# jkflying/opencalibration

Hardware: AMD Instinct MI355X
Metric: images/sec end-to-end (extract+match+relax) on synthetic aerial grid; LM iters/sec (higher is better)
Workload: dtype f32 (extract) + fp4 0/1 bits, f32 accumulate, exact (match) + f64 (RANSAC, relax)

## Files before the change

### opencalibration_amd/csrc/akaze.hip

```cpp
#include "area_table.hpp"
#include "ctx.hpp"

#include <algorithm>
#include <cmath>
#include <limits>
#include <cstring>
#include <type_traits>
#include <vector>

namespace
{

struct level_info
{
    int octave, w, h, sigma_size;
    float esigma;
    size_t off;
    int tile_off, tiles_x;
    int mask_off;
    int sup_off, sup_tx;
};

__device__ __forceinline__ int clampi(int v, int lo, int hi)
{
// ... 2655 lines not shown
    if (!ctx || !images_dev || !cams || !model3 || !plane2 || !lattice3)
        return OCHIP_EINVAL;
    if (n_images == 0)
        return OCHIP_OK;
    OCHIP_HIP(ctx, hipSetDevice(ctx->device));
    std::vector<synth_cam> hc(n_images);
    for (uint32_t i = 0; i < n_images; i++)
    {
        for (int k = 0; k < 3; k++)
            hc[i].pos[k] = (float)cams[7 * i + k];
        for (int k = 0; k < 4; k++)
            hc[i].q[k] = (float)cams[7 * i + 3 + k];
    }
    synth_cam *dc = nullptr;
    if (hipMalloc((void **)&dc, n_images * sizeof(synth_cam)) != hipSuccess)
        return ochip_fail(ctx, OCHIP_ENOMEM, "hipMalloc failed");
    hipError_t e = hipMemcpy(dc, hc.data(), n_images * sizeof(synth_cam), hipMemcpyHostToDevice);
    if (e == hipSuccess)
    {
        hipLaunchKernelGGL(render_views_kernel, dim3((width + 255) / 256, height, n_images), dim3(256), 0, ctx->stream,
                           images_dev + (size_t)first_image * width * height * 3, width, height, (const synth_cam *)dc,
                           (float)model3[0], (float)model3[1], (float)model3[2], (float)plane2[0], (float)plane2[1],
                           (float)lattice3[0], (float)lattice3[1], (float)lattice3[2], seed);
        e = ochip_stream_wait(ctx, ctx->stream);
    }
    (void)hipFree(dc);
    if (e != hipSuccess)
        return ochip_fail(ctx, OCHIP_EHIP, "ochip_synth_render_views: %s", hipGetErrorString(e));
    return OCHIP_OK;
}

}

namespace
{

const gather_tab &host_gather_tab()
{
    static const gather_tab G = []() {
        gather_tab T{};
        static const float gauss25[7][7] = {{0.02546481f, 0.02350698f, 0.01849125f, 0.01239505f, 0.00708017f, 0.00344629f, 0.00142946f},
                                            {0.02350698f, 0.02169968f, 0.01706957f, 0.01144208f, 0.00653582f, 0.00318132f, 0.00131956f},
                                            {0.01849125f, 0.01706957f, 0.01342740f, 0.00900066f, 0.00514126f, 0.00250252f, 0.00103800f},
                                            {0.01239505f, 0.01144208f, 0.00900066f, 0.00603332f, 0.00344629f, 0.00167749f, 0.00069579f},
                                            {0.00708017f, 0.00653582f, 0.00514126f, 0.00344629f, 0.00196855f, 0.00095820f, 0.00039744f},
                                            {0.00344629f, 0.00318132f, 0.00250252f, 0.00167749f, 0.00095820f, 0.00046640f, 0.00019346f},
                                            {0.00142946f, 0.00131956f, 0.00103800f, 0.00069579f, 0.00039744f, 0.00019346f, 0.00008024f}};
        std::vector<float> gw(169);
        for (int i = -6; i <= 6; i++)
            for (int j = -6; j <= 6; j++)
                gw[(i + 6) * 13 + (j + 6)] = gauss25[std::abs(i)][std::abs(j)];
        struct os
        {
            int q, i, j;
        };
        std::vector<os> S;
        int q = 0;
        for (int i = -6; i <= 6; i++)
            for (int j = -6; j <= 6; j++)
                if (i * i + j * j < 36)
                    S.push_back({q++, i, j});
        std::sort(S.begin(), S.end(), [](const os &a, const os &b) { return a.j != b.j ? a.j < b.j : a.i < b.i; });
        for (int L = 0; L < 128; L++)
        {
            T.ori[L] = 0xFFFFFFFFu;
            T.ori_g[L] = 0.0f;
// ... 38 lines not shown
                if (i < 6)
                    k = i;
                for (int ch = 0; ch < 3; ch++)
                    T.bit_ofs[3 * i + ch] = (unsigned int)((cell_of(full[k][0], full[k][1]) * 3 + channel_of[ch]) * 4) |
                                            ((unsigned int)((cell_of(full[k][0], full[k][2]) * 3 + channel_of[ch]) * 4) << 16);
                for (int q = 0; q < 3; q++)
                    full[k][q] = full[162 - i - 1][q];
            }
        }
        for (int i = 0; i < 64; i++)
            T.chain[i] = 3u << 11;
        struct ch_t
        {
            int cls, first_cell, i, j, follows;
        };
        std::vector<ch_t> chains;
        for (int k = 0; k < 4; k++)
            chains.push_back({0, k, -10 + (k / 2) * 10, -10 + (k % 2) * 10, 0});
        for (int k = 0; k < 9; k += 2)
            chains.push_back({1, 4 + k, -10 + (k / 3) * 7, -10 + (k % 3) * 7, k == 2 ? 1 : 0});
        for (int k = 0; k < 16; k += 4)
            chains.push_back({2, 13 + k, -10 + (k / 4) * 5, -10, 0});
        for (size_t cidx = 0; cidx < chains.size(); cidx++)
            for (int ch = 0; ch < 3; ch++)
            {
                const ch_t &cc = chains[cidx];
                const unsigned int p0 = (unsigned int)((cc.i + 10) * 21 + (cc.j + 10));
                T.chain[3 * cidx + ch] = p0 | ((unsigned int)ch << 9) | ((unsigned int)cc.cls << 11) |
                                         ((unsigned int)cc.first_cell << 13) | ((unsigned int)cc.follows << 18);
            }
        return T;
    }();
    return G;
}

int akaze_run(ochip_ctx *ctx, const uint8_t *images_bgr, bool on_device, uint32_t n_images, int width, int height,
              uint32_t max_kp, float *kp6, uint64_t *desc, uint32_t *counts, int *work_wh, const ochip_feature_lists *lists,
              double nms_radius)
{
    if (!ctx || !counts || (n_images && (!images_bgr || (!lists && (!kp6 || !desc)))))
        return OCHIP_EINVAL;
    if (width <= 0 || height <= 0)
        return ochip_fail(ctx, OCHIP_EINVAL, "bad image size %d x %d", width, height);
    OCHIP_HIP(ctx, hipSetDevice(ctx->device));
    hipStream_t st = ctx->stream;
    const double scale = std::min(1.f, float(1600) / (float)std::max(width, height));
    const int W = (int)std::lrint(width * scale), H = (int)std::lrint(height * scale);
    if (work_wh)
    {
        work_wh[0] = W;
        work_wh[1] = H;
    }
    for (uint32_t i = 0; i < n_images; i++)
        counts[i] = 0;
    if (n_images == 0)
        return OCHIP_OK;

    const int omax = 4, nsub = 4;
    const float soffset = 1.6f, dfactor = 1.5f, dthreshold = 0.00005f;
    levels_dev LV{};
    std::vector<std::vector<float>> tsteps;
    size_t img_stride = 0;
    int n_tiles = 0;
    size_t mask_stride = 0;
    size_t sup_stride = 0;
    {
// ... 23 lines not shown
                l.sup_tx = (lw + 7) / 8;
                sup_stride += (size_t)l.sup_tx * ((lh + 7) / 8);
                etime.push_back(0.5f * (l.esigma * l.esigma));
            }
        }
        tsteps.resize(LV.n);
        for (int i = 1; i < LV.n; i++)
            tsteps[i] = fed_taus(etime[i] - etime[i - 1], 0.25f);
    }
    const size_t plane0 = (size_t)W * H;
    const uint32_t B = n_images;
    const uint32_t max_cands = std::max<uint32_t>(max_kp * 4, 1u << 16);

    ochip::dev_scratch mem{ctx, "akaze"};
    constexpr auto WAIT = ochip::copy_mode::enqueue_wait;
    int rc = OCHIP_OK;
#define AK(call)                                                                                                       \
    do                                                                                                                 \
    {                                                                                                                  \
        if (rc == OCHIP_OK)                                                                                            \
            rc = (call);                                                                                               \
    } while (0)
    uint8_t *d_bgr = nullptr, *d_gray = nullptr;
    float *d_img = nullptr, *d_flow = nullptr, *d_ping = nullptr;
    float2 *d_Lxy = nullptr;
    float2 *d_Fit = nullptr;
    float *d_Lt = nullptr, *d_Rmax = nullptr, *d_kc = nullptr,
          *d_kp = nullptr;
    unsigned int *d_hmax = nullptr, *d_hist = nullptr, *d_ncand = nullptr, *d_pmax = nullptr;
    cand_t *d_cands = nullptr;
    unsigned char *d_dead = nullptr, *d_valid = nullptr;
    unsigned long long *d_desc = nullptr, *d_descc = nullptr;
    float *d_kpc = nullptr;
    unsigned int *d_counts = nullptr, *d_tile_counts = nullptr, *d_tile_base = nullptr, *d_tile_seq = nullptr;
    unsigned long long *d_mask = nullptr, *d_vmask = nullptr, *d_kmask = nullptr, *d_pmask = nullptr, *d_rmask = nullptr;
    unsigned int *d_found = nullptr;
    unsigned int *d_level_first = nullptr;
    unsigned int *d_turns = nullptr, *d_waiting = nullptr;
    unsigned int *d_wbase = nullptr, *d_live = nullptr, *d_nlive = nullptr;
    gather_tab *d_gtab = nullptr;
    const size_t src_px = (size_t)width * height;
    auto tiles = [&](int w, int h) { return dim3(8 * ((((w + BT_X - 1) / BT_X) * ((h + BT_Y - 1) / BT_Y) + 7) / 8), 1, B); };
    auto det_tiles = [&](int w, int h) { return dim3(8 * ((((w + BT_X - 1) / BT_X) * ((h + DT_Y - 1) / DT_Y) + 7) / 8), 1, B); };
    const dim3 tiles0 = tiles(W, H);
    const int n_tiles0 = ((W + BT_X - 1) / BT_X) * ((H + BT_Y - 1) / BT_Y);
    if (on_device)
        d_bgr = const_cast<uint8_t *>(images_bgr);
    else
        AK(mem.upload(&d_bgr, images_bgr, (size_t)B * src_px * 3, WAIT));
    AK(mem.alloc<uint8_t>(&d_gray, (size_t)B * src_px + 4));
    AK(mem.alloc<float>(&d_img, (size_t)B * plane0));
    AK(mem.alloc<float>(&d_flow, (size_t)B * plane0));
    AK(mem.alloc<float>(&d_ping, (size_t)B * plane0));
    AK(mem.alloc<unsigned int>(&d_pmax, (size_t)B * n_tiles0));
    AK(mem.alloc<float>(&d_Lt, (size_t)B * img_stride));
    AK(mem.alloc<float2>(&d_Lxy, (size_t)B * img_stride));
    AK(mem.alloc<float2>(&d_Fit, (size_t)B * img_stride));
    AK(mem.alloc<float>(&d_Rmax, (size_t)B * img_stride));
    AK(mem.alloc<float>(&d_kc, B));
    AK(mem.alloc<unsigned int>(&d_hmax, B));
    AK(mem.alloc<unsigned int>(&d_hist, (size_t)B * 301));
    AK(mem.alloc<unsigned int>(&d_ncand, B));
    AK(mem.alloc<cand_t>(&d_cands, (size_t)B * max_cands));
    AK(mem.alloc<unsigned char>(&d_dead, (size_t)B * max_cands));
    AK(mem.alloc<unsigned char>(&d_valid, (size_t)B * max_cands));
    AK(mem.alloc<float>(&d_kp, (size_t)B * max_cands * 6));
    AK(mem.alloc<unsigned long long>(&d_desc, (size_t)B * max_cands * 8));
    AK(mem.alloc<float>(&d_kpc, (size_t)B * max_kp * 6));
    AK(mem.alloc<unsigned long long>(&d_descc, (size_t)B * max_kp * 8));
    AK(mem.alloc<unsigned int>(&d_counts, B));
    AK(mem.alloc<unsigned int>(&d_tile_counts, (size_t)B * n_tiles));
    AK(mem.alloc<unsigned int>(&d_tile_base, (size_t)B * n_tiles));
    AK(mem.alloc<unsigned long long>(&d_mask, (size_t)B * mask_stride));
    AK(mem.alloc<unsigned long long>(&d_vmask, (size_t)B * mask_stride));
    AK(mem.alloc<unsigned long long>(&d_kmask, (size_t)B * sup_stride));
    AK(mem.alloc<unsigned long long>(&d_pmask, (size_t)B * sup_stride));
    AK(mem.alloc<unsigned long long>(&d_rmask, (size_t)B * sup_stride));
    AK(mem.alloc<unsigned int>(&d_turns, (size_t)B * 2 * max_cands));
    AK(mem.alloc<unsigned int>(&d_waiting, (size_t)B * LV.n));
    AK(mem.alloc<unsigned int>(&d_level_first, (size_t)B * (LV.n + 1)));
    AK(mem.alloc<unsigned int>(&d_found, (size_t)B * max_cands));
    AK(mem.alloc<unsigned int>(&d_wbase, (size_t)B * mask_stride));
    AK(mem.alloc<unsigned int>(&d_live, (size_t)B * max_cands));
    AK(mem.alloc<unsigned int>(&d_nlive, B));
    {
        std::vector<std::pair<uint64_t, unsigned int>> keyed;
        keyed.reserve(n_tiles);
        auto spread = [](uint32_t v) {
            uint64_t x = v;
            x = (x | (x << 16)) & 0x0000FFFF0000FFFFull;
            x = (x | (x << 8)) & 0x00FF00FF00FF00FFull;
            x = (x | (x << 4)) & 0x0F0F0F0F0F0F0F0Full;
            x = (x | (x << 2)) & 0x3333333333333333ull;
            x = (x | (x << 1)) & 0x5555555555555555ull;
            return x;
        };
        for (int i = 0; i < LV.n; i++)
        {
            const level_info &l = LV.l[i];
            const int ty_n = (l.h + DT_Y - 1) / DT_Y;
            for (int ty = 0; ty < ty_n; ty++)
                for (int tx = 0; tx < l.tiles_x; tx++)
                    keyed.emplace_back(((uint64_t)i << 48) | spread((uint32_t)tx) | (spread((uint32_t)ty) << 1),
                                       (unsigned int)(l.tile_off + ty * l.tiles_x + tx));
        }
        std::sort(keyed.begin(), keyed.end());
        std::vector<unsigned int> seq(keyed.size());
        for (size_t i = 0; i < keyed.size(); i++)
            seq[i] = keyed[i].second;
        AK(mem.upload(&d_tile_seq, seq.data(), seq.size(), WAIT));
    }
    {
        AK(mem.upload(&d_gtab, &host_gather_tab(), 1, WAIT));
    }
    if (rc != OCHIP_OK)
    return rc;
    auto grid2 = [&](int w, int h) { return dim3((w + 255) / 256, h, B); };
    auto taps_of = [](const std::vector<float> &k) {
        taps_t t{};
        t.n = (int)k.size();
        for (int i = 0; i < t.n && i < MAX_TAPS; i++)
            t.k[i] = k[i];
        return t;
    };
    const taps_t g1 = taps_of(gaussian_taps(1.0f)), g0 = taps_of(gaussian_taps(soffset));
    if (g1.n != 5 || g0.n != 9)
    return ochip_fail(ctx, OCHIP_EINVAL, "akaze: unexpected Gaussian kernel sizes %d / %d", g1.n, g0.n);
    hipEvent_t e0, e1;
    ochip_prof_begin(ctx, OCHIP_K_AKAZE, &e0, &e1);

    const size_t n_px = (size_t)B * src_px;
    const bool resized = !(W == width && H == height);
    area_tab tx, ty;
    bool staged = false;
    if (resized)
    {
        tx = area_table(width, W, 1.0 / scale);
        ty = area_table(height, H, 1.0 / scale);
        staged = width % 4 == 0;
        for (int x0 = 0; x0 < W && staged; x0 += 256)
        {
            const int x1 = std::min(x0 + 256, W);
            const int c0 = tx.si[tx.off[x0]] & ~3, c1 = tx.si[tx.off[x1] - 1];
            staged = c1 - c0 + 1 <= RS_PITCH - 3;
            for (int x = x0; x < x1 && staged; x++)
                staged = tx.off[x + 1] - tx.off[x] <= RESIZE_MAX_TAPS;
        }
        for (int y0 = 0; y0 < H && staged; y0 += RESIZE_ROWS)
        {
            const int y1 = std::min(y0 + RESIZE_ROWS, H);
            staged = ty.si[ty.off[y1] - 1] - ty.si[ty.off[y0]] + 1 <= RS_ROWS;
        }
    }
    const bool fused_grey = staged && ((uintptr_t)d_bgr & 3) == 0;
    if (!fused_grey)
    {
        if (((uintptr_t)d_bgr & 3) == 0)
            hipLaunchKernelGGL(gray4_kernel, dim3((unsigned)(((n_px + 3) / 4 + 255) / 256)), dim3(256), 0, st,
                               (const uint32_t *)d_bgr, (uint32_t *)d_gray, n_px / 4);
        if (((uintptr_t)d_bgr & 3) != 0 || (n_px & 3))
        {
            const size_t first = ((uintptr_t)d_bgr & 3) ? 0 : (n_px & ~(size_t)3);
            hipLaunchKernelGGL(gray_kernel, dim3((unsigned)((n_px - first + 255) / 256)), dim3(256), 0, st, d_bgr + 3 * first,
                               d_gray + first, n_px - first);
        }
    }
    if (W == width && H == height)
        hipLaunchKernelGGL(to_float_kernel, dim3((unsigned)((B * plane0 + 255) / 256)), dim3(256), 0, st, d_gray, d_img,
                           B * plane0);
    else
    {
        int *xo, *xs, *yo, *ys;
        float *xa, *ya;
        AK(mem.upload(&xo, tx.off.data(), tx.off.size(), WAIT));
        AK(mem.upload(&xs, tx.si.data(), tx.si.size(), WAIT));
        AK(mem.upload(&xa, tx.alpha.data(), tx.alpha.size(), WAIT));
        AK(mem.upload(&yo, ty.off.data(), ty.off.size(), WAIT));
        AK(mem.upload(&ys, ty.si.data(), ty.si.size(), WAIT));
        AK(mem.upload(&ya, ty.alpha.data(), ty.alpha.size(), WAIT));
        if (rc != OCHIP_OK)
        return rc;
        const dim3 rgrid((W + 255) / 256, (H + RESIZE_ROWS - 1) / RESIZE_ROWS, B);
        int most_taps = 0;
        for (int x = 0; x < W; x++)
            most_taps = std::max(most_taps, tx.off[x + 1] - tx.off[x]);
        const int half_up_cols = scale == 0.5 ? W - W % 16 : 0;
        if (fused_grey && most_taps <= 4)
            hipLaunchKernelGGL((resize_area_lds_kernel<true, 4>), rgrid, dim3(256), 0, st, (const uint8_t *)d_bgr, width, height, d_img,
                               W, H, xo, xs, xa, yo, ys, ya, half_up_cols);
        else if (fused_grey)
            hipLaunchKernelGGL((resize_area_lds_kernel<true, RESIZE_MAX_TAPS>), rgrid, dim3(256), 0, st, (const uint8_t *)d_bgr, width, height, d_img,
                               W, H, xo, xs, xa, yo, ys, ya, half_up_cols);
        else if (staged)
            hipLaunchKernelGGL((resize_area_lds_kernel<false, RESIZE_MAX_TAPS>), rgrid, dim3(256), 0, st, d_gray, width, height, d_img, W, H, xo, xs,
                               xa, yo, ys, ya, half_up_cols);
        else
            hipLaunchKernelGGL(resize_area_kernel, rgrid, dim3(256), 0, st, d_gray, width, height, d_img, W, H, xo, xs, xa, yo, ys,
                               ya, half_up_cols);
    }

    OCHIP_HIP(ctx, hipMemsetAsync(d_hist, 0, (size_t)B * 301 * 4, st));
    const bool modg_tiles = ochip_test_hook("tile_levels"), modg_force = ochip_test_hook("strip_levels");
    const bool modg_strip = !modg_tiles && (W & 1) == 0 && (plane0 & 1) == 0 && W >= 64 && H >= 64 && ((uintptr_t)d_img & 15) == 0 &&
                            ((uintptr_t)d_flow & 15) == 0 && (modg_force || (size_t)W * H * B >= ((size_t)32 << 20));
    if (modg_strip)
    {
        OCHIP_HIP(ctx, hipMemsetAsync(d_hmax, 0, (size_t)B * 4, st));
        level_strip_args sa{};
        sa.in = d_img, sa.in_stride = plane0;
        sa.flow = d_flow, sa.flow_stride = plane0;
        sa.w = W, sa.h = H;
        sa.hmax_bits = d_hmax;
        for (int q = 0; q < 5; q++)
            sa.k[q] = g1.k[q];
        typedef level_strip_geom<2, 0> MG;
        const int strips = ((W + MG::OW - 1) / MG::OW) * ((H + MG::H - 1) / MG::H);
        hipLaunchKernelGGL((level_strip_kernel<2, 0, true, true>), dim3(8 * (((strips + 3) / 4 + 7) / 8), 1, B), dim3(256), 0, st, sa);
    }
// ... 426 lines not shown
```

### opencalibration_amd/csrc/ctx.hip

```cpp
#include "ctx.hpp"

#include <cstring>

static std::string g_create_error;

int ochip_fail(ochip_ctx *ctx, int code, const char *fmt, ...)
{
    char buf[512];
    va_list ap;
    va_start(ap, fmt);
    vsnprintf(buf, sizeof buf, fmt, ap);
    va_end(ap);
    if (ctx)
        ctx->error = buf;
    else
        g_create_error = buf;
    return code;
}

int ochip_ensure(ochip_ctx *ctx, void **ptr, size_t *cap, size_t bytes)
{
    if (bytes <= *cap)
        return OCHIP_OK;
    if (*ptr)
// ... 78 lines not shown
        ochip_fail(ctx, OCHIP_ENOMEM, "device allocation of %zu bytes failed in %s", bytes, what);
    return d;
}

int dev_blocks::upload_bytes(void **dst, const void *src, size_t bytes, copy_mode m)
{
    void *d = get(bytes);
    if (!d)
        return OCHIP_ENOMEM;
    if (src && bytes)
    {
        hipError_t e = m == copy_mode::blocking ? hipMemcpy(d, src, bytes, hipMemcpyHostToDevice)
                                                : hipMemcpyAsync(d, src, bytes, hipMemcpyHostToDevice, ctx->stream);
        if (e == hipSuccess && m == copy_mode::enqueue_wait)
            e = ochip_stream_wait(ctx, ctx->stream);
        if (e != hipSuccess)
            return ochip_fail(ctx, OCHIP_EHIP, "host-to-device copy of %zu bytes failed in %s: %s", bytes, what, hipGetErrorString(e));
    }
    *dst = d;
    return OCHIP_OK;
}

void dev_blocks::release()
{
    for (auto &b : held)
        ochip_pool_put(ctx, b.first, b.second);
    held.clear();
}

dev_scratch::~dev_scratch()
{
    if (held.empty())
        return;
    (void)ochip_stream_wait(ctx, ctx->stream);
    release();
}
}

void ochip_prof_begin(ochip_ctx *ctx, int kid, hipEvent_t *start, hipEvent_t *stop)
{
    auto &s = ctx->prof[kid];
    if (!s.free_list.empty())
    {
        *start = s.free_list.back().first;
        *stop = s.free_list.back().second;
        s.free_list.pop_back();
    }
    else
    {
        (void)hipEventCreate(start);
        (void)hipEventCreate(stop);
    }
    (void)hipEventRecord(*start, ctx->stream);
}

static void prof_drain(ochip_ctx *ctx, int kid)
{
    auto &s = ctx->prof[kid];
    for (auto &p : s.pending)
    {
        float ms = 0;
        (void)hipEventSynchronize(p.second);
        if (hipEventElapsedTime(&ms, p.first, p.second) == hipSuccess)
        {
            s.total_ms += ms;
            s.launches++;
        }
        s.free_list.push_back(p);
    }
    s.pending.clear();
}

void ochip_prof_end(ochip_ctx *ctx, int kid, hipEvent_t start, hipEvent_t stop)
{
    (void)hipEventRecord(stop, ctx->stream);
    auto &s = ctx->prof[kid];
    s.pending.emplace_back(start, stop);
    if (s.pending.size() >= 4096)
        prof_drain(ctx, kid);
}

extern "C"
{

int ochip_ctx_create(int device, ochip_ctx **out)
{
    if (!out)
        return ochip_fail(nullptr, OCHIP_EINVAL, "out is NULL");
    *out = nullptr;
    int count = 0;
    if (hipGetDeviceCount(&count) != hipSuccess || count <= 0)
        return ochip_fail(nullptr, OCHIP_ENODEV, "no HIP device visible");
    if (device < 0 || device >= count)
        return ochip_fail(nullptr, OCHIP_EINVAL, "device %d out of range (0..%d)", device, count - 1);
    ochip_ctx *ctx = new (std::nothrow) ochip_ctx();
    if (!ctx)
        return ochip_fail(nullptr, OCHIP_ENOMEM, "host allocation failed");
    ctx->device = device;
    hipError_t e = hipSetDevice(device);
    const char *bsync = getenv("OCHIP_BLOCKING_SYNC");
    ctx->blocking_wait = !(bsync && bsync[0] == '0');
    if (e == hipSuccess && ctx->blocking_wait)
    {
        (void)hipSetDeviceFlags(hipDeviceScheduleBlockingSync);
        (void)hipGetLastError();
    }
    if (e == hipSuccess)
        e = hipGetDeviceProperties(&ctx->prop, device);
    if (e == hipSuccess && std::strncmp(ctx->prop.gcnArchName, "gfx950", 6) != 0)
    {
        int rc = ochip_fail(nullptr, OCHIP_ENODEV, "device %d is %s; libochip is built for gfx950 only", device,
                            ctx->prop.gcnArchName);
        delete ctx;
        return rc;
    }
    if (e == hipSuccess)
        e = hipStreamCreateWithFlags(&ctx->stream, hipStreamNonBlocking);
    if (e != hipSuccess)
    {
        int rc = ochip_fail(nullptr, OCHIP_EHIP, "context creation failed: %s", hipGetErrorString(e));
        delete ctx;
        return rc;
    }
    *out = ctx;
    return OCHIP_OK;
}

void ochip_ctx_destroy(ochip_ctx *ctx)
{
    if (!ctx)
        return;
    if (ctx->attachment && ctx->attachment_destroy)
        ctx->attachment_destroy(ctx->attachment);
    ctx->attachment = nullptr;
    for (ochip_ctx *sib : ctx->siblings)
        ochip_ctx_destroy(sib);
    ctx->siblings.clear();
    (void)hipSetDevice(ctx->device);
    (void)hipDeviceSynchronize();
    for (auto &s : ctx->prof)
    {
        for (auto &p : s.pending)
            s.free_list.push_back(p);
        for (auto &p : s.free_list)
        {
            (void)hipEventDestroy(p.first);
            (void)hipEventDestroy(p.second);
        }
    }
    void *bufs[] = {ctx->desc_dev,      ctx->img_off_dev,   ctx->img_n_dev, ctx->pairs_dev,    ctx->out_off_dev,
                    ctx->match_out_dev, ctx->kp_xy_dev,     ctx->rays_dev,  ctx->kp_image_dev, ctx->models_dev,
                    ctx->ms_recs_dev,   ctx->ms_seg_dev,    ctx->ms_flag_dev};
    for (void *b : bufs)
        if (b)
            (void)hipFree(b);
    for (void *b : ctx->scratch_dev)
        if (b)
            (void)hipFree(b);
    if (ctx->sym_jobs_dev)
        (void)hipFree(ctx->sym_jobs_dev);
    if (ctx->sym_part_dev)
        (void)hipFree(ctx->sym_part_dev);
    for (void *b : {ctx->desc_fp4_dev, ctx->desc_negpop_dev, ctx->desc_pop_dev})
        if (b)
            (void)hipFree(b);
    if (ctx->lab_table_mem)
    {
        ctx->lab_table_mem->release();
        delete ctx->lab_table_mem;
    }
    for (auto &b : ctx->dev_pool)
        (void)hipFree(b.first);
    for (auto &b : ctx->pinned_pool)
        (void)hipHostFree(b.first);
    for (auto &b : ctx->pinned_live)
        (void)hipHostFree(b.first);
    if (ctx->sync_event)
        (void)hipEventDestroy(ctx->sync_event);
    for (hipStream_t r : ctx->retired_streams)
        (void)hipStreamDestroy(r);
    if (ctx->stream)
        (void)hipStreamDestroy(ctx->stream);
    if (ctx->copy_stream)
        (void)hipStreamDestroy(ctx->copy_stream);
    delete ctx;
}

int ochip_ctx_set_priority(ochip_ctx *ctx, int high)
{
    if (!ctx)
        return OCHIP_EINVAL;
    if (ctx->stream_priority == (high ? 1 : 0))
        return OCHIP_OK;
    OCHIP_HIP(ctx, hipSetDevice(ctx->device));
    int least = 0, greatest = 0;
    OCHIP_HIP(ctx, hipDeviceGetStreamPriorityRange(&least, &greatest));
    OCHIP_HIP(ctx, hipStreamSynchronize(ctx->stream));
    hipStream_t s = nullptr;
    OCHIP_HIP(ctx, hipStreamCreateWithPriority(&s, hipStreamNonBlocking, high ? greatest : least));
    ctx->retired_streams.push_back(ctx->stream);
    ctx->stream = s;
    ctx->stream_priority = high ? 1 : 0;
    return OCHIP_OK;
}

int ochip_ctx_sibling(ochip_ctx *ctx, uint32_t index, ochip_ctx **out)
{
    if (!ctx || !out)
        return OCHIP_EINVAL;
    *out = nullptr;
    std::lock_guard<std::mutex> lock(ctx->siblings_mutex);
    if (index > 64)
        return ochip_fail(ctx, OCHIP_EINVAL, "sibling index %u out of range", index);
    while (ctx->siblings.size() <= index)
    {
        ochip_ctx *s = nullptr;
        const int rc = ochip_ctx_create(ctx->device, &s);
        if (rc != OCHIP_OK)
            return ochip_fail(ctx, rc, "sibling context: %s", ochip_last_error(nullptr));
        ctx->siblings.push_back(s);
    }
    *out = ctx->siblings[index];
    return OCHIP_OK;
}

void *ochip_ctx_attachment(ochip_ctx *ctx, void *(*make)(void), void (*destroy)(void *))
{
    if (!ctx)
        return nullptr;
    std::lock_guard<std::mutex> lock(ctx->siblings_mutex);
    if (!ctx->attachment && make)
    {
        ctx->attachment = make();
        ctx->attachment_destroy = destroy;
    }
    return ctx->attachment;
}

uint64_t ochip_akaze_progress(const ochip_ctx *ctx)
{
    return ctx ? ctx->akaze_readbacks.load(std::memory_order_acquire) : 0;
}

const char *ochip_last_error(const ochip_ctx *ctx)
{
    return ctx ? ctx->error.c_str() : g_create_error.c_str();
}

int ochip_device_info(const ochip_ctx *ctx, char *name, size_t name_len, int *compute_units, size_t *hbm_bytes)
{
    if (!ctx)
        return OCHIP_EINVAL;
    if (name && name_len)
        snprintf(name, name_len, "%s (%s)", ctx->prop.name[0] ? ctx->prop.name : "AMD Instinct (name table not installed)",
                 ctx->prop.gcnArchName);
    if (compute_units)
        *compute_units = ctx->prop.multiProcessorCount;
    if (hbm_bytes)
        *hbm_bytes = ctx->prop.totalGlobalMem;
    return OCHIP_OK;
}

int ochip_synchronize(ochip_ctx *ctx)
{
    if (!ctx)
        return OCHIP_EINVAL;
    OCHIP_HIP(ctx, ochip_stream_wait(ctx, ctx->stream));
    if (ctx->copy_stream)
        OCHIP_HIP(ctx, ochip_stream_wait(ctx, ctx->copy_stream));
    return OCHIP_OK;
}

int ochip_descriptors_reserve(ochip_ctx *ctx, uint32_t n_images, uint64_t total_descriptors)
{
    if (!ctx)
        return OCHIP_EINVAL;
    OCHIP_HIP(ctx, hipSetDevice(ctx->device));
    OCHIP_HIP(ctx, ochip_stream_wait(ctx, ctx->stream));
    ctx->kp_set.clear();
    ctx->rays_dirty = false;
    ctx->kp_store_ready = false;
    ctx->desc_capacity = ctx->desc_used = 0;
    ctx->fp4_valid = 0;
    ctx->n_images = n_images;
    ctx->img_off.assign(n_images, 0);
    ctx->img_n.assign(n_images, 0);
    ctx->img_set.assign(n_images, 0);
    ctx->img_tables_dirty = true;
    const size_t n_img = n_images ? n_images : 1;
    int rc = ochip_ensure(ctx, (void **)&ctx->desc_dev, &ctx->desc_bytes, (size_t)(total_descriptors ? total_descriptors : 1) * 64);
    if (rc == OCHIP_OK)
        rc = ochip_ensure(ctx, (void **)&ctx->img_off_dev, &ctx->img_off_bytes, n_img * 8);
    if (rc == OCHIP_OK)
        rc = ochip_ensure(ctx, (void **)&ctx->img_n_dev, &ctx->img_n_bytes, n_img * 4);
    if (rc != OCHIP_OK)
        return rc;
    ctx->desc_capacity = total_descriptors;
    return OCHIP_OK;
}

// ... 97 lines not shown
{
    if (!ctx || !p)
        return;
    for (size_t i = 0; i < ctx->pinned_live.size(); i++)
        if (ctx->pinned_live[i].first == p)
        {
            ctx->pinned_pool.push_back(ctx->pinned_live[i]);
            ctx->pinned_live.erase(ctx->pinned_live.begin() + i);
            while (ctx->pinned_pool.size() > 16)
            {
                size_t s = 0;
                for (size_t k = 1; k < ctx->pinned_pool.size(); k++)
                    if (ctx->pinned_pool[k].second < ctx->pinned_pool[s].second)
                        s = k;
                (void)hipHostFree(ctx->pinned_pool[s].first);
                ctx->pinned_pool.erase(ctx->pinned_pool.begin() + s);
            }
            return;
        }
}

int ochip_descriptor_count(const ochip_ctx *ctx, uint32_t image_id, uint32_t *n)
{
    if (!ctx || !n || image_id >= ctx->n_images || !ctx->img_set[image_id])
        return OCHIP_EINVAL;
    *n = ctx->img_n[image_id];
    return OCHIP_OK;
}

int ochip_profile_reset(ochip_ctx *ctx)
{
    if (!ctx)
        return OCHIP_EINVAL;
    OCHIP_HIP(ctx, ochip_stream_wait(ctx, ctx->stream));
    for (int k = 0; k < OCHIP_K_COUNT; k++)
    {
        prof_drain(ctx, k);
        ctx->prof[k].launches = 0;
        ctx->prof[k].total_ms = 0;
    }
    ctx->match_computed = ctx->match_delivered = 0;
    ctx->relax_mfma_flops = 0;
    ctx->ransac_hyp_corr = ctx->relax_blocks_jac = ctx->relax_blocks_cost = 0;
    for (ochip_ctx *sib : ctx->siblings)
    {
        const int rc = ochip_profile_reset(sib);
        if (rc != OCHIP_OK)
            return rc;
    }
    return OCHIP_OK;
}

int ochip_relax_work(ochip_ctx *ctx, double *mfma_flops)
{
    if (!ctx || !mfma_flops)
        return OCHIP_EINVAL;
    *mfma_flops = ctx->relax_mfma_flops;
    for (ochip_ctx *sib : ctx->siblings)
        *mfma_flops += sib->relax_mfma_flops;
    return OCHIP_OK;
}

int ochip_work_counters(ochip_ctx *ctx, uint64_t *counters3)
{
    if (!ctx || !counters3)
        return OCHIP_EINVAL;
    counters3[0] = ctx->ransac_hyp_corr;
// ... 73 lines not shown
```

### opencalibration_amd/csrc/ctx.hpp

```cpp
#pragma once

#include <hip/hip_runtime.h>

#include <atomic>
#include <cstdarg>
#include <cstdio>
#include <mutex>
#include <string>
#include <vector>

#include "../../include/ochip.h"
#include "env.hpp"

struct ochip_profile_slot
{
    std::vector<std::pair<hipEvent_t, hipEvent_t>> pending;
    std::vector<std::pair<hipEvent_t, hipEvent_t>> free_list;
    uint64_t launches = 0;
    double total_ms = 0;
};

namespace ochip
{
struct dev_blocks;
}

struct ochip_ctx
{
    int device = 0;
    hipStream_t stream = nullptr;
    hipStream_t copy_stream = nullptr;
    std::vector<hipStream_t> retired_streams;
    int stream_priority = -1;
    hipEvent_t sync_event = nullptr;
    bool blocking_wait = true;
    std::string error;
    hipDeviceProp_t prop{};

    uint32_t *desc_dev = nullptr;
    uint64_t desc_capacity = 0, desc_used = 0;
    uint32_t n_images = 0;
    std::vector<uint64_t> img_off;
    std::vector<uint32_t> img_n;
    std::vector<uint8_t> img_set;
    uint64_t *img_off_dev = nullptr;
    uint32_t *img_n_dev = nullptr;
    bool img_tables_dirty = true;

    double *kp_xy_dev = nullptr;
    double *rays_dev = nullptr;
    uint32_t *kp_image_dev = nullptr;
    double *models_dev = nullptr;
    std::vector<uint8_t> kp_set;
    bool rays_dirty = false;
    bool kp_store_ready = false;
    size_t desc_bytes = 0, img_off_bytes = 0, img_n_bytes = 0, kp_xy_bytes = 0, rays_bytes = 0, kp_image_bytes = 0,
           models_bytes = 0;

    ochip_pair *pairs_dev = nullptr;
    uint64_t *out_off_dev = nullptr;
    size_t pairs_cap = 0;
    ochip_match *match_out_dev = nullptr;
    size_t match_out_cap = 0;
    uint64_t match_out_total = 0;
    void *ms_recs_dev = nullptr, *ms_seg_dev = nullptr, *ms_flag_dev = nullptr;
    size_t ms_recs_cap = 0, ms_seg_cap = 0, ms_flag_cap = 0;
    uint32_t ms_pairs = 0;
    void *sym_jobs_dev = nullptr, *sym_part_dev = nullptr;
    size_t sym_jobs_cap = 0, sym_part_cap = 0;
    void *desc_fp4_dev = nullptr, *desc_negpop_dev = nullptr, *desc_pop_dev = nullptr;
    size_t desc_fp4_cap = 0, desc_negpop_cap = 0, desc_pop_cap = 0;
    uint64_t fp4_valid = 0;

    void *scratch_dev[8] = {nullptr};
    size_t scratch_cap[8] = {0};

    std::vector<std::pair<void *, size_t>> pinned_live, pinned_pool;
    std::vector<std::pair<void *, size_t>> dev_pool;

    ochip_profile_slot prof[OCHIP_K_COUNT];
    uint64_t match_computed = 0, match_delivered = 0;
    double relax_mfma_flops = 0;
    uint64_t ransac_hyp_corr = 0, relax_blocks_jac = 0, relax_blocks_cost = 0;
    uint64_t relax_system_bytes = 0, relax_system_dense_bytes = 0, relax_system_unknowns = 0;

    std::vector<ochip_ctx *> siblings;
    std::mutex siblings_mutex;

    std::atomic<uint64_t> akaze_readbacks{0};

    ochip::dev_blocks *lab_table_mem = nullptr;
    uint32_t *lab_table_dev = nullptr;
    void *lab_tables_dev = nullptr;
    float lab_table_fill_ms = 0;

    void *attachment = nullptr;
    void (*attachment_destroy)(void *) = nullptr;
};


inline hipError_t ochip_stream_wait(ochip_ctx *ctx, hipStream_t st)
{
    if (!ctx->blocking_wait)
        return hipStreamSynchronize(st);
    if (!ctx->sync_event)
    {
        const hipError_t e = hipEventCreateWithFlags(&ctx->sync_event, hipEventBlockingSync | hipEventDisableTiming);
        if (e != hipSuccess)
            return e;
    }
    const hipError_t e = hipEventRecord(ctx->sync_event, st);
    return e != hipSuccess ? e : hipEventSynchronize(ctx->sync_event);
}

inline hipError_t ochip_copy_stream(ochip_ctx *ctx, hipStream_t *out)
{
    hipError_t e = hipSuccess;
    if (!ctx->copy_stream)
        e = hipStreamCreateWithFlags(&ctx->copy_stream, hipStreamNonBlocking);
    *out = ctx->copy_stream;
    return e;
}

int ochip_fail(ochip_ctx *ctx, int code, const char *fmt, ...);
int ochip_ensure(ochip_ctx *ctx, void **ptr, size_t *cap, size_t bytes);
int ochip_ensure_keypoint_store(ochip_ctx *ctx, size_t n_keypoints, size_t n_images);
void *ochip_pool_get(ochip_ctx *ctx, size_t bytes, size_t *got);
void ochip_pool_put(ochip_ctx *ctx, void *p, size_t bytes);
void ochip_prof_begin(ochip_ctx *ctx, int kid, hipEvent_t *start, hipEvent_t *stop);
void ochip_prof_end(ochip_ctx *ctx, int kid, hipEvent_t start, hipEvent_t stop);

#define OCHIP_HIP(ctx, call)                                                                                           \
    do                                                                                                                 \
    {                                                                                                                  \
        hipError_t e__ = (call);                                                                                       \
// ... 72 lines not shown
```

### opencalibration_amd/csrc/host/extract_features.cpp

```cpp
#include "../env.hpp"
#include "extract_features.hpp"
#include "extract_slots.hpp"
#include "sort_like_std.hpp"

#include <algorithm>
#include <chrono>
#include <cmath>
#include <condition_variable>
#include <cstdio>
#include <cstdlib>
#include <cstring>
#include <deque>
#include <limits>
#include <mutex>
#include <thread>

#include <emmintrin.h>
#include <omp.h>

namespace opencalibration_amd
{

namespace
{
// ... 268 lines not shown
            g_tail_prof[i] += d[i];
        }
    }
}

struct chunk_buffers
{
    float *kp = nullptr;
    uint64_t *desc = nullptr;
    uint8_t *prepared = nullptr;
    ochip_feature_lists lists{};
    std::vector<uint32_t> counts;
    uint32_t first = 0, n = 0;
};

extract_slots &slots_of(ochip_ctx *root)
{
    void *p = ochip_ctx_attachment(
        root, []() -> void * { return new extract_slots(); }, [](void *q) { delete static_cast<extract_slots *>(q); });
    return *static_cast<extract_slots *>(p);
}

extract_slots::order handover_order()
{
    const char *gate = std::getenv("OCHIP_EXTRACT_GATE");
    if (gate && gate[0] == '0')
        return extract_slots::order::none;
    const char *e = std::getenv("OCHIP_EXTRACT_HANDOVER");
    if (e && std::strcmp(e, "survey") == 0)
        return extract_slots::order::survey;
    return extract_slots::order::slot;
}

bool stagger_starts()
{
    const char *e = std::getenv("OCHIP_EXTRACT_STAGGER");
    return e && e[0] == '1';
}
}

uint32_t extract_chunk_size()
{
    if (const char *e = std::getenv("OCHIP_EXTRACT_CHUNK"))
    {
        const long v = std::atol(e);
        if (v >= 1 && v <= 1024)
            return (uint32_t)v;
    }
    return 100;
}

std::vector<extracted_features> extract_features_batch(ochip_ctx *ctx, const uint8_t *images_bgr, uint32_t n_images,
                                                       int width, int height, uint32_t max_keypoints, std::string *error,
                                                       bool images_on_device)
{
    std::vector<extracted_features> out(n_images);
    const bool ok = extract_features_stream(ctx, images_bgr, n_images, width, height, max_keypoints, images_on_device, 0,
                                            [&](uint32_t first, uint32_t count, extracted_features *f) {
                                                for (uint32_t i = 0; i < count; i++)
                                                    out[first + i] = std::move(f[i]);
                                            },
                                            error);
    if (!ok)
        return {};
    return out;
}

bool extract_features_stream(ochip_ctx *ctx, const uint8_t *images_bgr, uint32_t n_images, int width, int height,
                             uint32_t max_keypoints, bool images_on_device, int host_threads,
                             const std::function<void(uint32_t, uint32_t, extracted_features *)> &on_chunk,
                             std::string *error, extract_timing *timing)
{
    if (timing)
        *timing = extract_timing{};
    if (n_images == 0)
        return true;
    if (width <= 0 || height <= 0)
    {
        std::vector<extracted_features> empty(n_images);
        on_chunk(0, n_images, empty.data());
        return true;
    }
    const int tail_threads = host_threads > 0 ? host_threads : omp_get_max_threads();
    const int max_length_pixels = 1600;
    const double scale = std::min(1.f, float(max_length_pixels) / (float)std::max(width, height));
    const uint32_t host_chunk = 25;
    const uint32_t chunk = std::min(images_on_device ? extract_chunk_size() : host_chunk, n_images);
    const size_t image_bytes = (size_t)width * height * 3;

    uint32_t n_drivers = images_on_device ? 4 : 5;
    if (const char *e = std::getenv("OCHIP_EXTRACT_STREAMS"))
        n_drivers = (uint32_t)std::max(1L, std::min(5L, std::atol(e)));
    const uint32_t n_chunks = (n_images + chunk - 1) / chunk;
    n_drivers = std::min(n_drivers, n_chunks);
    std::vector<ochip_ctx *> ctxs(n_drivers, ctx);
    for (uint32_t d = 1; d < n_drivers; d++)
        if (ochip_ctx_sibling(ctx, d - 1, &ctxs[d]) != OCHIP_OK)
        {
            if (error)
                *error = std::string("ochip_ctx_sibling: ") + ochip_last_error(ctx);
            return false;
        }
    const bool device_tail = !ochip_test_hook("host_tail");
    const double nms_pixel_radius = 8;
    const bool force_host_nms = ochip_test_hook("host_nms");
    extract_slots &slots = slots_of(ctx);
    const extract_slots::order handover = handover_order();
    const auto t_enter = std::chrono::steady_clock::now();
    extract_ticket ticket(slots, n_drivers);
    constexpr int BPS = extract_slots::BUFFERS_PER_SLOT;
    const uint32_t n_bufs = BPS * n_drivers;
    std::vector<chunk_buffers> bufs(n_bufs);
    std::string fail;
    const size_t rows = (size_t)chunk * max_keypoints;
    const size_t o_resp = (rows + chunk) * 88, o_slot = o_resp + rows * 4, o_ns = o_slot + rows * 4, o_conf = o_ns + (size_t)chunk * 4;
    const size_t pad = ((size_t)chunk + 15) / 16 * 16;
    const size_t o_sub = o_conf + pad, o_nsub = o_sub + (size_t)chunk * OCHIP_SUBSET_CAP * 4, o_sconf = o_nsub + (size_t)chunk * 4;
    const size_t want[2] = {device_tail ? o_sconf + pad : rows * 6 * sizeof(float), device_tail ? 0 : rows * 8 * sizeof(uint64_t)};
    auto shape_buffer = [&](ochip_ctx *dctx, extract_slots::buffer &sb, chunk_buffers &b) -> bool {
        const int layout = device_tail ? 0 : 1;
        if (sb.layout != layout || sb.bytes[0] < want[0] || sb.bytes[1] < want[1])
        {
            for (int k = 0; k < 2; k++)
            {
                if (sb.block[k])
                    ochip_host_free(dctx, sb.block[k]);
                sb.block[k] = nullptr;
                sb.bytes[k] = 0;
            }
            sb.layout = -1;
// ... 30 lines not shown
    };
    double tail_cpu_seconds = 0;
    std::mutex mu;
    std::condition_variable cv;
    std::deque<int> ready;
    uint32_t next_chunk = 0, drivers_done = 0;
    bool started = false;
    std::chrono::steady_clock::time_point t_first_slot = t_enter;
    const bool stagger = stagger_starts();
    const bool trace = ochip_verbose("extract");
    std::vector<uint64_t> progress_at_start(n_drivers, 0);
    std::vector<char> in_first_phase(n_drivers, 0);

    std::vector<double> driver_cpu(n_drivers, 0.0);
    auto driver = [&](uint32_t d) {
        ochip_ctx *dctx = ctxs[d];
        const double cpu0 = thread_cpu_now();
        struct at_exit
        {
            double &out, t0;
            ~at_exit() { out = thread_cpu_now() - t0; }
        } record{driver_cpu[d], cpu0};
        {
            slot_hold hold(slots, ticket.id(), d, handover);
            if (trace)
                fprintf(stderr, "[extract] survey %llu driver %u: slot acquired\n", (unsigned long long)ticket.id(), d);
            {
                std::lock_guard<std::mutex> lk(mu);
                if (!started)
                {
                    started = true;
                    t_first_slot = std::chrono::steady_clock::now();
                }
            }
            for (;;)
            {
                uint32_t c = 0;
                bool go = false;
                {
                    std::unique_lock<std::mutex> lk(mu);
                    if (stagger)
                        while (fail.empty() && next_chunk < n_chunks)
                        {
                            bool other = false;
                            for (uint32_t o = 0; o < n_drivers; o++)
                                if (o != d && in_first_phase[o])
                                {
                                    if (ochip_akaze_progress(ctxs[o]) != progress_at_start[o])
                                        in_first_phase[o] = 0;
                                    else
                                        other = true;
                                }
                            if (!other)
                                break;
                            cv.wait_for(lk, std::chrono::milliseconds(1));
                        }
                    if (fail.empty() && next_chunk < n_chunks)
                    {
                        c = next_chunk++;
                        go = true;
                        if (stagger)
                        {
                            progress_at_start[d] = ochip_akaze_progress(dctx);
                            in_first_phase[d] = 1;
                        }
                    }
// ... 185 lines not shown
```

Baseline: 3831.

## Cache AKAZE lookup tables per context and give extract drivers their own streams

The tile-order sequence, gather table and area-resize tables are now built and uploaded once per context and reused while the image geometry stays the same. Previously they were rebuilt and uploaded with blocking copies on every akaze_run call. Context streams are now created lazily, so a priority change before first use does not create and retire a stream. Extraction drivers now all use dedicated sibling contexts set to low priority, keeping extraction off the caller's stream. The cost is extra per-context state and a priority class that may change how extraction overlaps with matching and relaxation work.

```diff
diff --git a/opencalibration_amd/csrc/akaze.hip b/opencalibration_amd/csrc/akaze.hip
--- a/opencalibration_amd/csrc/akaze.hip
+++ b/opencalibration_amd/csrc/akaze.hip
@@ -2711,6 +2711,18 @@
 
 }
 
+struct ochip::akaze_tables
+{
+    ochip::dev_blocks mem;
+    int width = 0, height = 0, W = 0, H = 0, n_levels = 0, n_tiles = 0;
+    unsigned int *tile_seq = nullptr;
+    void *gtab = nullptr;
+    int *xo = nullptr, *xs = nullptr, *yo = nullptr, *ys = nullptr;
+    float *xa = nullptr, *ya = nullptr;
+    bool staged = false;
+    int most_taps = 0;
+};
+
 namespace
 {
 
@@ -2815,6 +2827,93 @@
         return T;
     }();
     return G;
+}
+
+int akaze_tables_for(ochip_ctx *ctx, int width, int height, int W, int H, double scale, const levels_dev &LV, int n_tiles,
+                     const ochip::akaze_tables **out)
+{
+    if (!ctx->akaze_tabs)
+    {
+        ctx->akaze_tabs = new ochip::akaze_tables();
+        ctx->akaze_tabs->mem.ctx = ctx;
+        ctx->akaze_tabs->mem.what = "akaze tables";
+        ctx->akaze_tabs_destroy = [](ochip::akaze_tables *t) {
+            t->mem.release();
+            delete t;
+        };
+    }
+    ochip::akaze_tables &T = *ctx->akaze_tabs;
+    *out = &T;
+    if (T.width == width && T.height == height && T.W == W && T.H == H && T.n_levels == LV.n && T.n_tiles == n_tiles)
+        return OCHIP_OK;
+    T.width = 0;
+    T.mem.release();
+    constexpr auto ENQ = ochip::copy_mode::enqueue;
+    int rc = OCHIP_OK;
+    std::vector<std::pair<uint64_t, unsigned int>> keyed;
+    keyed.reserve(n_tiles);
+    auto spread = [](uint32_t v) {
+        uint64_t x = v;
+        x = (x | (x << 16)) & 0x0000FFFF0000FFFFull;
+        x = (x | (x << 8)) & 0x00FF00FF00FF00FFull;
+        x = (x | (x << 4)) & 0x0F0F0F0F0F0F0F0Full;
+        x = (x | (x << 2)) & 0x3333333333333333ull;
+        x = (x | (x << 1)) & 0x5555555555555555ull;
+        return x;
+    };
+    for (int i = 0; i < LV.n; i++)
+    {
+        const level_info &l = LV.l[i];
+        const int ty_n = (l.h + DT_Y - 1) / DT_Y;
+        for (int ty = 0; ty < ty_n; ty++)
+            for (int tx = 0; tx < l.tiles_x; tx++)
+                keyed.emplace_back(((uint64_t)i << 48) | spread((uint32_t)tx) | (spread((uint32_t)ty) << 1),
+                                   (unsigned int)(l.tile_off + ty * l.tiles_x + tx));
+    }
+    std::sort(keyed.begin(), keyed.end());
+    std::vector<unsigned int> seq(keyed.size());
+    for (size_t i = 0; i < keyed.size(); i++)
+        seq[i] = keyed[i].second;
+    rc = rc != OCHIP_OK ? rc : T.mem.upload(&T.tile_seq, seq, ENQ);
+    gather_tab *g = nullptr;
+    rc = rc != OCHIP_OK ? rc : T.mem.upload(&g, &host_gather_tab(), 1, ENQ);
+    T.gtab = g;
+    area_tab tx, ty;
+    T.staged = false;
+    T.most_taps = 0;
+    if (!(W == width && H == height))
+    {
+        tx = area_table(width, W, 1.0 / scale);
+        ty = area_table(height, H, 1.0 / scale);
+        bool staged = width % 4 == 0;
+        for (int x0 = 0; x0 < W && staged; x0 += 256)
+        {
+            const int x1 = std::min(x0 + 256, W);
+            const int c0 = tx.si[tx.off[x0]] & ~3, c1 = tx.si[tx.off[x1] - 1];
+            staged = c1 - c0 + 1 <= RS_PITCH - 3;
+            for (int x = x0; x < x1 && staged; x++)
+                staged = tx.off[x + 1] - tx.off[x] <= RESIZE_MAX_TAPS;
+        }
+        for (int y0 = 0; y0 < H && staged; y0 += RESIZE_ROWS)
+        {
+            const int y1 = std::min(y0 + RESIZE_ROWS, H);
+            staged = ty.si[ty.off[y1] - 1] - ty.si[ty.off[y0]] + 1 <= RS_ROWS;
+        }
+        T.staged = staged;
+        for (int x = 0; x < W; x++)
+            T.most_taps = std::max(T.most_taps, tx.off[x + 1] - tx.off[x]);
+        rc = rc != OCHIP_OK ? rc : T.mem.upload(&T.xo, tx.off, ENQ);
+        rc = rc != OCHIP_OK ? rc : T.mem.upload(&T.xs, tx.si, ENQ);
+        rc = rc != OCHIP_OK ? rc : T.mem.upload(&T.xa, tx.alpha, ENQ);
+        rc = rc != OCHIP_OK ? rc : T.mem.upload(&T.yo, ty.off, ENQ);
+        rc = rc != OCHIP_OK ? rc : T.mem.upload(&T.ys, ty.si, ENQ);
+        rc = rc != OCHIP_OK ? rc : T.mem.upload(&T.ya, ty.alpha, ENQ);
+    }
+    OCHIP_HIP(ctx, ochip_stream_wait(ctx, ctx->stream));
+    if (rc != OCHIP_OK)
+        return rc;
+    T.width = width, T.height = height, T.W = W, T.H = H, T.n_levels = LV.n, T.n_tiles = n_tiles;
+    return OCHIP_OK;
 }
 
 int akaze_run(ochip_ctx *ctx, const uint8_t *images_bgr, bool on_device, uint32_t n_images, int width, int height,
@@ -2904,13 +3003,12 @@
     unsigned char *d_dead = nullptr, *d_valid = nullptr;
     unsigned long long *d_desc = nullptr, *d_descc = nullptr;
     float *d_kpc = nullptr;
-    unsigned int *d_counts = nullptr, *d_tile_counts = nullptr, *d_tile_base = nullptr, *d_tile_seq = nullptr;
+    unsigned int *d_counts = nullptr, *d_tile_counts = nullptr, *d_tile_base = nullptr;
     unsigned long long *d_mask = nullptr, *d_vmask = nullptr, *d_kmask = nullptr, *d_pmask = nullptr, *d_rmask = nullptr;
     unsigned int *d_found = nullptr;
     unsigned int *d_level_first = nullptr;
     unsigned int *d_turns = nullptr, *d_waiting = nullptr;
     unsigned int *d_wbase = nullptr, *d_live = nullptr, *d_nlive = nullptr;
-    gather_tab *d_gtab = nullptr;
     const size_t src_px = (size_t)width * height;
     auto tiles = [&](int w, int h) { return dim3(8 * ((((w + BT_X - 1) / BT_X) * ((h + BT_Y - 1) / BT_Y) + 7) / 8), 1, B); };
     auto det_tiles = [&](int w, int h) { return dim3(8 * ((((w + BT_X - 1) / BT_X) * ((h + DT_Y - 1) / DT_Y) + 7) / 8), 1, B); };
@@ -2955,38 +3053,12 @@
     AK(mem.alloc<unsigned int>(&d_wbase, (size_t)B * mask_stride));
     AK(mem.alloc<unsigned int>(&d_live, (size_t)B * max_cands));
     AK(mem.alloc<unsigned int>(&d_nlive, B));
-    {
-        std::vector<std::pair<uint64_t, unsigned int>> keyed;
-        keyed.reserve(n_tiles);
-        auto spread = [](uint32_t v) {
-            uint64_t x = v;
-            x = (x | (x << 16)) & 0x0000FFFF0000FFFFull;
-            x = (x | (x << 8)) & 0x00FF00FF00FF00FFull;
-            x = (x | (x << 4)) & 0x0F0F0F0F0F0F0F0Full;
-            x = (x | (x << 2)) & 0x3333333333333333ull;
-            x = (x | (x << 1)) & 0x5555555555555555ull;
-            return x;
-        };
-        for (int i = 0; i < LV.n; i++)
-        {
-            const level_info &l = LV.l[i];
-            const int ty_n = (l.h + DT_Y - 1) / DT_Y;
-            for (int ty = 0; ty < ty_n; ty++)
-                for (int tx = 0; tx < l.tiles_x; tx++)
-                    keyed.emplace_back(((uint64_t)i << 48) | spread((uint32_t)tx) | (spread((uint32_t)ty) << 1),
-                                       (unsigned int)(l.tile_off + ty * l.tiles_x + tx));
-        }
-        std::sort(keyed.begin(), keyed.end());
-        std::vector<unsigned int> seq(keyed.size());
-        for (size_t i = 0; i < keyed.size(); i++)
-            seq[i] = keyed[i].second;
-        AK(mem.upload(&d_tile_seq, seq.data(), seq.size(), WAIT));
-    }
-    {
-        AK(mem.upload(&d_gtab, &host_gather_tab(), 1, WAIT));
-    }
+    const ochip::akaze_tables *tabs = nullptr;
+    AK(akaze_tables_for(ctx, width, height, W, H, scale, LV, n_tiles, &tabs));
     if (rc != OCHIP_OK)
     return rc;
+    const unsigned int *d_tile_seq = tabs->tile_seq;
+    const gather_tab *d_gtab = (const gather_tab *)tabs->gtab;
     auto grid2 = [&](int w, int h) { return dim3((w + 255) / 256, h, B); };
     auto taps_of = [](const std::vector<float> &k) {
         taps_t t{};
@@ -3003,27 +3075,7 @@
 
     const size_t n_px = (size_t)B * src_px;
     const bool resized = !(W == width && H == height);
-    area_tab tx, ty;
-    bool staged = false;
-    if (resized)
-    {
-        tx = area_table(width, W, 1.0 / scale);
-        ty = area_table(height, H, 1.0 / scale);
-        staged = width % 4 == 0;
-        for (int x0 = 0; x0 < W && staged; x0 += 256)
-        {
-            const int x1 = std::min(x0 + 256, W);
-            const int c0 = tx.si[tx.off[x0]] & ~3, c1 = tx.si[tx.off[x1] - 1];
-            staged = c1 - c0 + 1 <= RS_PITCH - 3;
-            for (int x = x0; x < x1 && staged; x++)
-                staged = tx.off[x + 1] - tx.off[x] <= RESIZE_MAX_TAPS;
-        }
-        for (int y0 = 0; y0 < H && staged; y0 += RESIZE_ROWS)
-        {
-            const int y1 = std::min(y0 + RESIZE_ROWS, H);
-            staged = ty.si[ty.off[y1] - 1] - ty.si[ty.off[y0]] + 1 <= RS_ROWS;
-        }
-    }
+    const bool staged = resized && tabs->staged;
     const bool fused_grey = staged && ((uintptr_t)d_bgr & 3) == 0;
     if (!fused_grey)
     {
@@ -3042,20 +3094,10 @@
                            B * plane0);
     else
     {
-        int *xo, *xs, *yo, *ys;
-        float *xa, *ya;
-        AK(mem.upload(&xo, tx.off.data(), tx.off.size(), WAIT));
-        AK(mem.upload(&xs, tx.si.data(), tx.si.size(), WAIT));
-        AK(mem.upload(&xa, tx.alpha.data(), tx.alpha.size(), WAIT));
-        AK(mem.upload(&yo, ty.off.data(), ty.off.size(), WAIT));
-        AK(mem.upload(&ys, ty.si.data(), ty.si.size(), WAIT));
-        AK(mem.upload(&ya, ty.alpha.data(), ty.alpha.size(), WAIT));
-        if (rc != OCHIP_OK)
-        return rc;
+        const int *xo = tabs->xo, *xs = tabs->xs, *yo = tabs->yo, *ys = tabs->ys;
+        const float *xa = tabs->xa, *ya = tabs->ya;
         const dim3 rgrid((W + 255) / 256, (H + RESIZE_ROWS - 1) / RESIZE_ROWS, B);
-        int most_taps = 0;
-        for (int x = 0; x < W; x++)
-            most_taps = std::max(most_taps, tx.off[x + 1] - tx.off[x]);
+        const int most_taps = tabs->most_taps;
         const int half_up_cols = scale == 0.5 ? W - W % 16 : 0;
         if (fused_grey && most_taps <= 4)
             hipLaunchKernelGGL((resize_area_lds_kernel<true, 4>), rgrid, dim3(256), 0, st, (const uint8_t *)d_bgr, width, height, d_img,
diff --git a/opencalibration_amd/csrc/ctx.hip b/opencalibration_amd/csrc/ctx.hip
--- a/opencalibration_amd/csrc/ctx.hip
+++ b/opencalibration_amd/csrc/ctx.hip
@@ -134,9 +134,31 @@
 {
     if (held.empty())
         return;
-    (void)ochip_stream_wait(ctx, ctx->stream);
+    if (ctx->stream.opened())
+        (void)ochip_stream_wait(ctx, ctx->stream);
     release();
 }
+}
+
+void ochip_lazy_stream::open()
+{
+    int current = -1;
+    error = hipGetDevice(&current);
+    if (error == hipSuccess && current != device)
+        error = hipSetDevice(device);
+    if (error == hipSuccess && priority < 0)
+        error = hipStreamCreateWithFlags(&s, hipStreamNonBlocking);
+    else if (error == hipSuccess)
+    {
+        int least = 0, greatest = 0;
+        error = hipDeviceGetStreamPriorityRange(&least, &greatest);
+        if (error == hipSuccess)
+            error = hipStreamCreateWithPriority(&s, hipStreamNonBlocking, priority ? greatest : least);
+    }
+    if (current >= 0 && current != device)
+        (void)hipSetDevice(current);
+    if (error != hipSuccess)
+        s = nullptr;
 }
 
 void ochip_prof_begin(ochip_ctx *ctx, int kid, hipEvent_t *start, hipEvent_t *stop)
@@ -198,7 +220,7 @@
     ochip_ctx *ctx = new (std::nothrow) ochip_ctx();
     if (!ctx)
         return ochip_fail(nullptr, OCHIP_ENOMEM, "host allocation failed");
-    ctx->device = device;
+    ctx->device = ctx->stream.device = device;
     hipError_t e = hipSetDevice(device);
     const char *bsync = getenv("OCHIP_BLOCKING_SYNC");
     ctx->blocking_wait = !(bsync && bsync[0] == '0');
@@ -216,8 +238,6 @@
         delete ctx;
         return rc;
     }
-    if (e == hipSuccess)
-        e = hipStreamCreateWithFlags(&ctx->stream, hipStreamNonBlocking);
     if (e != hipSuccess)
     {
         int rc = ochip_fail(nullptr, OCHIP_EHIP, "context creation failed: %s", hipGetErrorString(e));
@@ -266,6 +286,9 @@
     for (void *b : {ctx->desc_fp4_dev, ctx->desc_negpop_dev, ctx->desc_pop_dev})
         if (b)
             (void)hipFree(b);
+    if (ctx->akaze_tabs && ctx->akaze_tabs_destroy)
+        ctx->akaze_tabs_destroy(ctx->akaze_tabs);
+    ctx->akaze_tabs = nullptr;
     if (ctx->lab_table_mem)
     {
         ctx->lab_table_mem->release();
@@ -281,8 +304,8 @@
         (void)hipEventDestroy(ctx->sync_event);
     for (hipStream_t r : ctx->retired_streams)
         (void)hipStreamDestroy(r);
-    if (ctx->stream)
-        (void)hipStreamDestroy(ctx->stream);
+    if (ctx->stream.opened())
+        (void)hipStreamDestroy(ctx->stream.s);
     if (ctx->copy_stream)
         (void)hipStreamDestroy(ctx->copy_stream);
     delete ctx;
@@ -294,15 +317,20 @@
         return OCHIP_EINVAL;
     if (ctx->stream_priority == (high ? 1 : 0))
         return OCHIP_OK;
+    if (!ctx->stream.opened())
+    {
+        ctx->stream.priority = ctx->stream_priority = high ? 1 : 0;
+        return OCHIP_OK;
+    }
     OCHIP_HIP(ctx, hipSetDevice(ctx->device));
     int least = 0, greatest = 0;
     OCHIP_HIP(ctx, hipDeviceGetStreamPriorityRange(&least, &greatest));
     OCHIP_HIP(ctx, hipStreamSynchronize(ctx->stream));
     hipStream_t s = nullptr;
     OCHIP_HIP(ctx, hipStreamCreateWithPriority(&s, hipStreamNonBlocking, high ? greatest : least));
-    ctx->retired_streams.push_back(ctx->stream);
-    ctx->stream = s;
-    ctx->stream_priority = high ? 1 : 0;
+    ctx->retired_streams.push_back(ctx->stream.s);
+    ctx->stream.s = s;
+    ctx->stream.priority = ctx->stream_priority = high ? 1 : 0;
     return OCHIP_OK;
 }
 
@@ -367,7 +395,10 @@
 {
     if (!ctx)
         return OCHIP_EINVAL;
-    OCHIP_HIP(ctx, ochip_stream_wait(ctx, ctx->stream));
+    if (ctx->stream.opened())
+        OCHIP_HIP(ctx, ochip_stream_wait(ctx, ctx->stream));
+    else if (ctx->stream.error != hipSuccess)
+        OCHIP_HIP(ctx, ctx->stream.error);
     if (ctx->copy_stream)
         OCHIP_HIP(ctx, ochip_stream_wait(ctx, ctx->copy_stream));
     return OCHIP_OK;
@@ -531,7 +562,8 @@
 {
     if (!ctx)
         return OCHIP_EINVAL;
-    OCHIP_HIP(ctx, ochip_stream_wait(ctx, ctx->stream));
+    if (ctx->stream.opened())
+        OCHIP_HIP(ctx, ochip_stream_wait(ctx, ctx->stream));
     for (int k = 0; k < OCHIP_K_COUNT; k++)
     {
         prof_drain(ctx, k);
diff --git a/opencalibration_amd/csrc/ctx.hpp b/opencalibration_amd/csrc/ctx.hpp
--- a/opencalibration_amd/csrc/ctx.hpp
+++ b/opencalibration_amd/csrc/ctx.hpp
@@ -25,10 +25,38 @@
 struct dev_blocks;
 }
 
+struct ochip_lazy_stream
+{
+    hipStream_t s = nullptr;
+    int device = 0;
+    int priority = -1;
+    hipError_t error = hipSuccess;
+
+    ochip_lazy_stream() = default;
+    ochip_lazy_stream(const ochip_lazy_stream &) = delete;
+    ochip_lazy_stream &operator=(const ochip_lazy_stream &) = delete;
+    bool opened() const
+    {
+        return s != nullptr;
+    }
+    operator hipStream_t()
+    {
+        if (!s)
+            open();
+        return s;
+    }
+    void open();
+};
+
+namespace ochip
+{
+struct akaze_tables;
+}
+
 struct ochip_ctx
 {
     int device = 0;
-    hipStream_t stream = nullptr;
+    ochip_lazy_stream stream;
     hipStream_t copy_stream = nullptr;
     std::vector<hipStream_t> retired_streams;
     int stream_priority = -1;
@@ -94,6 +122,9 @@
     void *lab_tables_dev = nullptr;
     float lab_table_fill_ms = 0;
 
+    ochip::akaze_tables *akaze_tabs = nullptr;
+    void (*akaze_tabs_destroy)(ochip::akaze_tables *) = nullptr;
+
     void *attachment = nullptr;
     void (*attachment_destroy)(void *) = nullptr;
 };
@@ -101,6 +132,8 @@
 
 inline hipError_t ochip_stream_wait(ochip_ctx *ctx, hipStream_t st)
 {
+    if (ctx->stream.error != hipSuccess)
+        return ctx->stream.error;
     if (!ctx->blocking_wait)
         return hipStreamSynchronize(st);
     if (!ctx->sync_event)
diff --git a/opencalibration_amd/csrc/host/extract_features.cpp b/opencalibration_amd/csrc/host/extract_features.cpp
--- a/opencalibration_amd/csrc/host/extract_features.cpp
+++ b/opencalibration_amd/csrc/host/extract_features.cpp
@@ -324,6 +324,12 @@
     return extract_slots::order::slot;
 }
 
+bool own_stream_class()
+{
+    const char *e = std::getenv("OCHIP_EXTRACT_PRIORITY");
+    return !(e && e[0] == '0');
+}
+
 bool stagger_starts()
 {
     const char *e = std::getenv("OCHIP_EXTRACT_STAGGER");
@@ -385,9 +391,11 @@
         n_drivers = (uint32_t)std::max(1L, std::min(5L, std::atol(e)));
     const uint32_t n_chunks = (n_images + chunk - 1) / chunk;
     n_drivers = std::min(n_drivers, n_chunks);
+    constexpr uint32_t FIRST_SLOT_SIBLING = 21;
+    const bool own_class = own_stream_class();
     std::vector<ochip_ctx *> ctxs(n_drivers, ctx);
-    for (uint32_t d = 1; d < n_drivers; d++)
-        if (ochip_ctx_sibling(ctx, d - 1, &ctxs[d]) != OCHIP_OK)
+    for (uint32_t d = own_class ? 0 : 1; d < n_drivers; d++)
+        if (ochip_ctx_sibling(ctx, own_class ? FIRST_SLOT_SIBLING + d : d - 1, &ctxs[d]) != OCHIP_OK)
         {
             if (error)
                 *error = std::string("ochip_ctx_sibling: ") + ochip_last_error(ctx);
@@ -484,6 +492,13 @@
                     started = true;
                     t_first_slot = std::chrono::steady_clock::now();
                 }
+            }
+            if (own_class && ochip_ctx_set_priority(dctx, 0) != OCHIP_OK)
+            {
+                std::lock_guard<std::mutex> lk(mu);
+                if (fail.empty())
+                    fail = std::string("ochip_ctx_set_priority: ") + ochip_last_error(dctx);
+                ticket.retire();
             }
             for (;;)
             {
```

New measurement: 4047 (median of 6 runs). 5.6% higher.
